# Sukikui/PTI-LDM-VAE

Hardware: AMD Instinct MI355X
Metric: vae_train_images_per_sec_256x256 (higher is better)
Workload: dtype fp16 forward operands + activations / bf16 backward operands + gradients, fp32 accumulate; 1 GPU; config/vae_dente_no_adv.json 256x256x1 batch 32/GPU: fwd + L1 + 1e-3*KL + bwd + all-reduce + Adam (perceptual term omitted: --perceptual times it; adversarial branch inactive before epoch 6, --adv times it); global_batch=32, parallelism=dp1

## Files before the change

pti_ldm_vae_amd/csrc/wgrad_mfma.hip:

```cpp
#include "pti_common.h"

namespace {

constexpr int TH = 8, TW = 16;
constexpr int PTI_WGRAD_SLAB_V4 = 1 << 30;
#ifndef PTI_WGRAD_BATCH_MAX
#define PTI_WGRAD_BATCH_MAX 16
#endif

struct WgArgs {
  const bf16* x;
  const bf16* dy;
  const stat_t* in_stats;
  const float* gamma;
  const float* beta;
  float* slab;
  int N, H, W, Cin, Ho, Wo, Cout;
  int mode, prologue, groups;
  float eps, inv_cnt;
  int tiles_x, tiles_y, ntiles, S;
  int ci_tiles;
  long long slab_stride;
  int x_f16;
  int diag;
};

template <int KS, int S_, int CO_T, int CI_T>
struct WCfg {
  static constexpr int HH = (TH - 1) * S_ + KS, HW = (TW - 1) * S_ + KS;
  static constexpr int NP = HH * HW;
  static constexpr int KK = KS * KS;
  static constexpr int PA = CI_T * 2 + (CI_T == 64 ? 64 : 0);
  static constexpr int PD = CO_T * 2 + (CO_T == 64 ? 64 : 0);
  static constexpr int NCA = CI_T / 8, NCD = CO_T / 8;
  static constexpr int WCO = CO_T / 32, WCI = CI_T / 32, WPX = 4 / (WCO * WCI);
  static constexpr int A_BYTES = NP * PA, D_BYTES = TH * TW * PD;
  static constexpr int HIT = (NP * NCA + 255) / 256, DIT = (TH * TW * NCD + 255) / 256;
  static constexpr int RED_BYTES = (WPX > 1) ? 32 * 32 * 4 * (WPX - 1) * WCO * WCI : 0;
  static constexpr int LDS_BYTES = (A_BYTES + D_BYTES) > RED_BYTES ? (A_BYTES + D_BYTES) : RED_BYTES;
};

template <int KS, int S_, int CO_T, int CI_T, bool PLAIN>
__global__ __launch_bounds__(256, 2) void wgrad_mfma_kernel(WgArgs a) {
  using C = WCfg<KS, S_, CO_T, CI_T>;
  const int prologue = PLAIN ? PTI_PRO_NONE : a.prologue;
  typedef short v4s __attribute__((ext_vector_type(4)));
  __shared__ __attribute__((aligned(16))) unsigned char smem[C::LDS_BYTES];
  unsigned char* lA = smem;
  unsigned char* lD = smem + C::A_BYTES;

  const int tid = threadIdx.x, lane = tid & 63, wave = tid >> 6;
  const int split = blockIdx.y;
// ... 370 lines not shown
#pragma unroll
          for (int h = 0; h < COB; ++h)
            acc[h][kh] = __builtin_amdgcn_mfma_f32_32x32x16_bf16(dfr[h][o], afr, acc[h][kh], 0, 0, 0);
        }
      }
    }
    __syncthreads();
  }

  float* slab = a.slab + (size_t)split * a.slab_stride;
  const int ci = cit * 32 + (lane & 31);
  const int hsel = lane >> 5;
#pragma unroll
  for (int h = 0; h < COB; ++h)
#pragma unroll
    for (int kh = 0; kh < 3; ++kh)
#pragma unroll
      for (int r = 0; r < 16; ++r) {
        const int co = co0 + h * 32 + (r & 3) + 8 * (r >> 2) + 4 * hsel;
        slab[((size_t)(kh * 3 + kw) * a.Cout + co) * a.Cin + ci] = acc[h][kh][r];
      }
  if (cit == 0) {
    float* red = reinterpret_cast<float*>(smem);
#pragma unroll
    for (int j = 0; j < 8; ++j) red[j * C::NT + tid] = bsum[j];
    __syncthreads();
    if (tid < 32 * COB) {
      const int c8 = tid / 8, j = tid % 8;
      float sm = 0.f;
      for (int k = c8; k < C::NT; k += C::DPC) sm += red[j * C::NT + k];
      slab[(size_t)9 * a.Cout * a.Cin + co0 + tid] = sm;
    }
  }
}

__device__ __attribute__((aligned(16))) unsigned int pti_wgrad_zero_page[4] = {0u, 0u, 0u, 0u};

__device__ __forceinline__ void glds16(const void* gsrc, unsigned lds_dst) {
  unsigned keep;
  asm volatile("s_mov_b32 %0, m0\n\ts_mov_b32 m0, %2\n\ts_nop 0\n\tglobal_load_lds_dwordx4 %1, off\n\ts_mov_b32 m0, %0"
               : "=&s"(keep) : "v"(gsrc), "s"(lds_dst) : "memory");
}
template <int N> __device__ __forceinline__ void wait_vmcnt() { asm volatile("s_waitcnt vmcnt(%0)" :: "n"(N) : "memory"); }

constexpr int W4_STG = 20 * 1024, W4_DP = 3, W4_NSTAGE = 2 * (W4_DP + 1), W4_IMG = 9 * 32 * 32 * 4;
constexpr int W4_STG2 = 28 * 1024, W4_DP2 = 4, W4_NST2 = W4_DP2 + 1;
constexpr int W4_LDS = (W4_NSTAGE * W4_STG > 4 * W4_IMG + 1024) ? W4_NSTAGE * W4_STG : 4 * W4_IMG + 1024;

struct W4Job {
  const bf16* x; const bf16* dy; float* slab;
  long long slab_stride;
  int N, H, W, Cin, Cout, tiles_x, tiles_y, ntiles, S;
  int cob2;
};
constexpr int W4_MAXGRP = 64;
struct W4Batch {
  W4Job job[PTI_WGRAD_BATCH_MAX];
  float* dw[PTI_WGRAD_BATCH_MAX];
  float* dbias[PTI_WGRAD_BATCH_MAX];
  int accumulate[PTI_WGRAD_BATCH_MAX];
  int first_rblk[PTI_WGRAD_BATCH_MAX + 1];
  unsigned short grp[8][W4_MAXGRP];
  unsigned short grp_start[8][W4_MAXGRP + 1];
  int ngrp[8];
  int njobs, diag, nwg;
};

static_assert(sizeof(W4Batch) <= 4096 && PTI_WGRAD_BATCH_MAX <= 16, "kernarg limit / 4-bit job index of the group word");

template <bool COB2>
__global__ __launch_bounds__(512, 1) void wgrad_mfma4_kernel(W4Batch b) {
  constexpr int HWp = TW + 2, NPX = 10 * HWp, PP = 64, XB = 12 * 1024, STG = W4_STG, DP = W4_DP, NPS = DP + 1;
  static_assert(W4_LDS <= 160 * 1024 && 5 * (DP - 1) <= 63, "ring must fit the LDS and the vmcnt counter");
  static_assert(W4_NST2 * W4_STG2 <= W4_LDS && 5 * (W4_DP2 - 1) <= 63, "two-block ring must fit as well");
  const int xcd = blockIdx.x & 7, pos = blockIdx.x >> 3;
  const int ng = b.ngrp[xcd];
  if (ng == 0 || pos >= b.grp_start[xcd][ng]) return;
  int gi = 0;
  while (gi + 1 < ng && pos >= b.grp_start[xcd][gi + 1]) ++gi;
  const unsigned gword = b.grp[xcd][gi];
  const int jb = gword & 15, split = gword >> 4, cc = pos - b.grp_start[xcd][gi];
  const W4Job& a = b.job[jb];
  const int ci_tiles = a.Cin / 32;
  typedef short v4s __attribute__((ext_vector_type(4)));
  typedef short v8s __attribute__((ext_vector_type(8)));
  __shared__ __attribute__((aligned(16))) unsigned char smem[W4_LDS];
  const unsigned lds0 = (unsigned)(size_t)(__attribute__((address_space(3))) unsigned char*)smem;
  const int tid = threadIdx.x, lane = tid & 63;
  const int w8 = __builtin_amdgcn_readfirstlane(tid >> 6);
  const int grp = w8 >> 2, w = w8 & 3;
  const int cot = cc / ci_tiles, cit = cc % ci_tiles;
  constexpr bool cob2 = COB2;
  const int co0 = cob2 ? (2 * cot + grp) * 32 : cot * 32, ci0 = cit * 32;
  const bool do_bias = (cit == 0);

  int xhy[3], xhx[3], xrel[3];
#pragma unroll
  for (int k = 0; k < 3; ++k) {
    const int i = (w + 4 * k) * 64 + lane, p = i >> 2;
    xhy[k] = p < NPX ? p / HWp : 1 << 20;
    xhx[k] = p - (p / HWp) * HWp;
    xrel[k] = ((xhy[k] - 1) * a.W + xhx[k] - 1) * a.Cin * 2 + (ci0 + (i & 3) * 8) * 2;
  }
  int dty[2], dtx[2], drel[2];
#pragma unroll
  for (int k = 0; k < 2; ++k) {
// ... 417 lines not shown
    for (int bl = 0; bl < 2; ++bl) {
      const float t = bsum[bl] + __shfl_xor(bsum[bl], 32, 64);
      if (lane < 32) bred[(w * 2 + bl) * 32 + lane] = t;
    }
  }
  if (w >= 2) { dump(red + (2 * (w - 2)) * 9216, 0); dump(red + (2 * (w - 2) + 1) * 9216, 1); }
  __syncthreads();
  if (w < 2) { gather(red + (2 * w) * 9216, 0); gather(red + (2 * w + 1) * 9216, 1); }
  __syncthreads();
  if (w == 1) { dump(red, 0); dump(red + 9216, 1); }
  __syncthreads();
  if (w == 0) { gather(red, 0); gather(red + 9216, 1); }
  __syncthreads();
  if (w == 0) { dump(red, 0); dump(red + 9216, 1); }
  __syncthreads();
  float* slab2 = a.slab + (size_t)split * a.slab_stride + (size_t)(2 * cot * ci_tiles + cit) * 9216;
  for (int i4 = tid; i4 < 2 * 2304; i4 += 256) {
    const int g2 = i4 >= 2304, j4 = i4 - g2 * 2304;
    *(f32x4*)(slab2 + (size_t)g2 * ci_tiles * 9216 + j4 * 4) = *(const f32x4*)(red + g2 * 9216 + j4 * 4);
  }
  if (do_bias && tid < 64) {
    const int g2 = tid >> 5;
    float sm = 0.f;
#pragma unroll
    for (int k = 0; k < 4; ++k) sm += bred[(k * 2 + g2) * 32 + (tid & 31)];
    a.slab[(size_t)split * a.slab_stride + (size_t)9 * a.Cout * a.Cin + cot * 64 + tid] = sm;
  }
#undef AC
}

template <int NCB_, int NCH_, int NRG_>
struct W6Cfg {
  static constexpr int NCB = NCB_, NCH = NCH_, NRG = NRG_, TH_ = 4 * NRG_, HW_ = TW + 2, NPX = (TH_ + 2) * HW_;
  static constexpr int XI = (NPX + 15) / 16;
  static constexpr int XSUB = XI * 1024, XB = NCH * XSUB, DSUB = TH_ * 1024, STG = XB + NCB * DSUB;
  static constexpr int NX = NCH * XI, KX = (NX + 7) / 8, ND = NCB * TH_, KD = ND / 8, NSLOT = KX + KD;
  static constexpr bool SINK = NX % 8 != 0;
  static constexpr int STGS = STG + (SINK ? 1024 : 0);
  static constexpr int FOLD = NRG == 2 ? NCB * NCH * 5 * 1024 * 4 + 1024 : 0;
#ifdef W6_NST3
  static constexpr int NST = 3, DP = 2;
#else
  static constexpr int NST = (124 * 1024) / STGS >= 4 ? 4 : 3, DP = NST - 1;
#endif
  static constexpr int LDS = NST * STGS > FOLD ? NST * STGS : FOLD;
  static_assert(NCB * NCH * NRG == 8 && ND % 8 == 0 && LDS <= 160 * 1024 && NSLOT * (DP - 1) <= 63, "v6 shape");
};
using W6A = W6Cfg<4, 2, 1>;
using W6B = W6Cfg<2, 2, 2>;

#ifndef W6_VGPR_ATTR
#define W6_VGPR_ATTR
#endif
template <class C>
__global__ W6_VGPR_ATTR __launch_bounds__(512, 1) void wgrad_mfma6_kernel(W4Batch b) {
  constexpr int PP = 64, HWp = C::HW_;
  const int xcd = blockIdx.x & 7, pos = blockIdx.x >> 3;
  const int ng = b.ngrp[xcd];
  if (ng == 0 || pos >= b.grp_start[xcd][ng]) return;
  int gi = 0;
  while (gi + 1 < ng && pos >= b.grp_start[xcd][gi + 1]) ++gi;
  const unsigned gword = b.grp[xcd][gi];
  const int jb = gword & 15, split = gword >> 4, cc = pos - b.grp_start[xcd][gi];
  const W4Job& a = b.job[jb];
  const int ci_pairs = a.Cin / (32 * C::NCH);
  typedef short v4s __attribute__((ext_vector_type(4)));
  typedef short v8s __attribute__((ext_vector_type(8)));
  __shared__ __attribute__((aligned(16))) unsigned char smem[C::LDS];
  const unsigned lds0 = (unsigned)(size_t)(__attribute__((address_space(3))) unsigned char*)smem;
  const int tid = threadIdx.x, lane = tid & 63;
  const int w8 = __builtin_amdgcn_readfirstlane(tid >> 6);
  const int cb = w8 % C::NCB, ch = (w8 / C::NCB) % C::NCH, rg = w8 / (C::NCB * C::NCH);
  const int cotb = cc / ci_pairs, citb = cc % ci_pairs;
  const int co0 = cotb * 32 * C::NCB, ci0 = citb * 32 * C::NCH;
  const bool do_bias = (citb == 0) && (ch == 0);

  int H = a.H, W = a.W;
  asm volatile("" : "+s"(H), "+s"(W));
  int ldsoff[C::NSLOT];
  int yy[C::NSLOT], xx[C::NSLOT], rel[C::NSLOT];
  bool pv[C::NSLOT];
  {
    const int pix = lane >> 2, piece = lane & 3;
#pragma unroll
    for (int k = 0; k < C::KX; ++k) {
      const int xi = w8 + 8 * k;
      const bool sink = xi >= C::NX;
      const int h = xi / C::XI, i = xi - C::XI * h, p = 16 * i + pix;
      ldsoff[k] = sink ? C::STG : h * C::XSUB + i * 1024;
      pv[k] = !sink && p < C::NPX;
      yy[k] = p / HWp - 1;
      xx[k] = p - (p / HWp) * HWp - 1;
      rel[k] = (yy[k] * W + xx[k]) * a.Cin * 2 + (ci0 + h * 32 + piece * 8) * 2;
    }
#pragma unroll
    for (int k = C::KX; k < C::NSLOT; ++k) {
      const int di = w8 + 8 * (k - C::KX), c = di / C::TH_, i = di % C::TH_;
      ldsoff[k] = C::XB + c * C::DSUB + i * 1024;
      pv[k] = true;
      yy[k] = i;
      xx[k] = pix;
      rel[k] = (i * W + pix) * a.Cout * 2 + (co0 + c * 32 + piece * 8) * 2;
    }
#pragma unroll
    for (int k = 0; k < C::NSLOT; ++k) ldsoff[k] = __builtin_amdgcn_readfirstlane(ldsoff[k]);
  }
  const unsigned char* xb = reinterpret_cast<const unsigned char*>(a.x);
  const unsigned char* db = reinterpret_cast<const unsigned char*>(a.dy);
  const unsigned char* zero = reinterpret_cast<const unsigned char*>(pti_wgrad_zero_page);
  struct TilePos { const unsigned char* xt; const unsigned char* dt; int oy0, ox0; };
  auto locate = [&](int tile) -> TilePos {
    TilePos tp;
    const bool live = tile < a.ntiles;
    int t = live ? tile : 0;
    const int tx_ = t % a.tiles_x; t /= a.tiles_x;
    const int ty_ = t % a.tiles_y;
    const int n = t / a.tiles_y;
    tp.oy0 = live ? ty_ * C::TH_ : 1 << 24; tp.ox0 = tx_ * TW;
    const size_t pix0 = (size_t)(n * H + ty_ * C::TH_) * W + tp.ox0;
    tp.xt = xb + pix0 * a.Cin * 2;
    tp.dt = db + pix0 * a.Cout * 2;
    return tp;
  };
  auto issue_slot = [&](const TilePos& tp, int stage, int k) {
    if (b.diag & 1) return;
    const unsigned sb = __builtin_amdgcn_readfirstlane(lds0 + stage * C::STGS + ldsoff[k]);
    const bool ok = pv[k] && (unsigned)(tp.oy0 + yy[k]) < (unsigned)H && (unsigned)(tp.ox0 + xx[k]) < (unsigned)W;
    glds16(ok ? (k < C::KX ? tp.xt : tp.dt) + rel[k] : zero, sb);
  };

  f32x16 acc[3][3];
  float bsum = 0.f;
#pragma unroll
  for (int r = 0; r < 16; ++r)
#pragma unroll
    for (int kh = 0; kh < 3; ++kh)
#pragma unroll
      for (int kw = 0; kw < 3; ++kw) acc[kh][kw][r] = 0.f;
  const int g = lane >> 4, q = (lane & 15) >> 2, pp = lane & 3;
  const int fbase = (8 * (g >> 1) + q) * PP + (16 * (g & 1) + 4 * pp) * 2;
  auto tr_frag = [&](const unsigned char* p) -> bf16x8 {
    const v4s d0 = __builtin_amdgcn_ds_read_tr16_b64_v4i16((v4s __attribute__((address_space(3)))*)(p));
    const v4s d1 = __builtin_amdgcn_ds_read_tr16_b64_v4i16((v4s __attribute__((address_space(3)))*)(p + 4 * PP));
    const v8s t = {d0[0], d0[1], d0[2], d0[3], d1[0], d1[1], d1[2], d1[3]};
    return __builtin_bit_cast(bf16x8, t);
  };

  const int ntl = a.ntiles > split ? (a.ntiles - split + a.S - 1) / a.S : 0;
  auto tile_of = [&](int k) { return k < ntl ? split + k * a.S : a.ntiles; };
#pragma unroll
  for (int s = 0; s < C::DP; ++s) {
    const TilePos tp = locate(tile_of(s));
#pragma unroll
    for (int k = 0; k < C::NSLOT; ++k) issue_slot(tp, s, k);
  }
  bf16x8 dfr[4], xcur, xq1;
  auto xfrag_at = [&](const unsigned char* lX, int f) { return tr_frag(lX + fbase + ((4 * rg + f / 3) * HWp + f % 3) * PP); };
  auto dfrag_at = [&](const unsigned char* lS, int r) { return tr_frag(lS + C::XB + cb * C::DSUB + fbase + (4 * rg + r) * TW * PP); };
  wait_vmcnt<C::NSLOT * (C::DP - 1)>();
  __builtin_amdgcn_s_barrier();
#pragma unroll
  for (int r = 0; r < 4; ++r) dfr[r] = dfrag_at(smem, r);
  xcur = xfrag_at(smem + ch * C::XSUB, 0);
  xq1 = xfrag_at(smem + ch * C::XSUB, 1);

  int ps = 0;
  for (int it = 0; it < ntl; ++it) {
    int fs = ps + C::DP;
    fs = fs >= C::NST ? fs - C::NST : fs;
    const int ns = ps + 1 == C::NST ? 0 : ps + 1;
    const TilePos ft = locate(tile_of(it + C::DP));
    wait_vmcnt<C::NSLOT * (C::DP - 2)>();
    __builtin_amdgcn_s_barrier();
    const unsigned char* lX = smem + ps * C::STGS + ch * C::XSUB;
    const unsigned char* lN = smem + ns * C::STGS;
    if (b.diag & 2) {
#pragma unroll
      for (int k = 0; k < C::NSLOT; ++k) issue_slot(ft, fs, k);
      ps = ns;
      continue;
    }
    if (do_bias) {
#pragma unroll
      for (int r = 0; r < 4; ++r) {
        const u32x4 dwv = __builtin_bit_cast(u32x4, dfr[r]);
        float s8 = 0.f;
#pragma unroll
        for (int i = 0; i < 4; ++i) s8 += __uint_as_float(dwv[i] << 16) + __uint_as_float(dwv[i] & 0xffff0000u);
        bsum += s8;
      }
    }
    bf16x8 dnx[4];
#pragma unroll
    for (int f = 0; f < 18; ++f) {
      const int rr = f / 3, kw = f % 3;
      bf16x8 xq2 = f + 2 < 18 ? xfrag_at(lX, f + 2) : xfrag_at(lN + ch * C::XSUB, f + 2 - 18);
      if (kw == 0 && rr >= 2) dnx[rr - 2] = dfrag_at(lN, rr - 2);
#pragma unroll
      for (int kh = 0; kh < 3; ++kh) {
        const int r = rr - kh;
        if (r >= 0 && r < 4) acc[kh][kw] = __builtin_amdgcn_mfma_f32_32x32x16_bf16(dfr[r], xcur, acc[kh][kw], 0, 0, 0);
      }
      if (C::NSLOT == 4) {
        if (f == 2) issue_slot(ft, fs, 0);
        if (f == 6) issue_slot(ft, fs, 1);
        if (f == 10) issue_slot(ft, fs, 2);
        if (f == 14) issue_slot(ft, fs, 3);
      } else {
        if (f == 2) issue_slot(ft, fs, 0);
        if (f == 5) issue_slot(ft, fs, 1);
        if (f == 8) issue_slot(ft, fs, 2);
        if (f == 11) issue_slot(ft, fs, 3);
        if (f == 14) issue_slot(ft, fs, C::NSLOT - 1);
      }
      if (kw == 0 && rr >= 2) __builtin_amdgcn_sched_group_barrier(0x100, 4, 0);
      else __builtin_amdgcn_sched_group_barrier(0x100, 2, 0);
      {
        const int nm = (rr == 0 || rr == 5) ? 1 : ((rr == 1 || rr == 4) ? 2 : 3);
        if (nm == 3) __builtin_amdgcn_sched_group_barrier(0x008, 3, 0);
        else if (nm == 2) __builtin_amdgcn_sched_group_barrier(0x008, 2, 0);
        else __builtin_amdgcn_sched_group_barrier(0x008, 1, 0);
      }
      __builtin_amdgcn_sched_barrier(0);
      xcur = xq1;
      xq1 = xq2;
    }
#pragma unroll
    for (int r = 0; r < 4; ++r) dfr[r] = dnx[r];
    ps = ns;
  }
  wait_vmcnt<0>();

  const int ci = lane & 31, hsel = lane >> 5;
  if (do_bias) bsum += __shfl_xor(bsum, 32, 64);
  if constexpr (C::NRG == 2) {
    __syncthreads();
    float* red = reinterpret_cast<float*>(smem) + (cb + C::NCB * ch) * 5120;
    float* bred = reinterpret_cast<float*>(smem) + C::NCB * C::NCH * 5120;
#pragma unroll
    for (int round = 0; round < 2; ++round) {
      if (round) __syncthreads();
      if (rg == 1) {
#pragma unroll
        for (int t = 0; t < 9; ++t)
          if ((t < 5) == (round == 0))
#pragma unroll
            for (int q4 = 0; q4 < 4; ++q4)
              *(f32x4*)(red + (t - 5 * round) * 1024 + ci * 32 + (((2 * q4 + hsel) ^ (ci & 7)) << 2)) =
                  f32x4{acc[t / 3][t % 3][4 * q4], acc[t / 3][t % 3][4 * q4 + 1], acc[t / 3][t % 3][4 * q4 + 2], acc[t / 3][t % 3][4 * q4 + 3]};
        if (round == 0 && do_bias && lane < 32) bred[cb * 32 + lane] = bsum;
      }
      __syncthreads();
      if (rg == 0) {
#pragma unroll
        for (int t = 0; t < 9; ++t)
          if ((t < 5) == (round == 0))
#pragma unroll
            for (int q4 = 0; q4 < 4; ++q4) {
              const f32x4 v = *(const f32x4*)(red + (t - 5 * round) * 1024 + ci * 32 + (((2 * q4 + hsel) ^ (ci & 7)) << 2));
#pragma unroll
              for (int j = 0; j < 4; ++j) acc[t / 3][t % 3][4 * q4 + j] += v[j];
            }
        if (round == 0 && do_bias && lane < 32) bsum += bred[cb * 32 + lane];
      }
    }
    if (rg == 1) return;
  }
  const int cc32 = (C::NCB * cotb + cb) * (a.Cin / 32) + C::NCH * citb + ch;
  float* blk = a.slab + (size_t)split * a.slab_stride + (size_t)cc32 * 9216;
#pragma unroll
  for (int kh = 0; kh < 3; ++kh)
#pragma unroll
    for (int kw = 0; kw < 3; ++kw)
#pragma unroll
      for (int q4 = 0; q4 < 4; ++q4)
        *(f32x4*)(blk + (kh * 3 + kw) * 1024 + ci * 32 + (((2 * q4 + hsel) ^ (ci & 7)) << 2)) =
            f32x4{acc[kh][kw][4 * q4], acc[kh][kw][4 * q4 + 1], acc[kh][kw][4 * q4 + 2], acc[kh][kw][4 * q4 + 3]};
  if (do_bias && lane < 32) a.slab[(size_t)split * a.slab_stride + (size_t)9 * a.Cout * a.Cin + co0 + cb * 32 + lane] = bsum;
}

__global__ __launch_bounds__(256) void wgrad_reduce4_kernel(W4Batch b) {
  __shared__ f32x4 red[16][16];
  int jb = 0;
  while (jb + 1 < b.njobs && (int)blockIdx.x >= b.first_rblk[jb + 1]) ++jb;
  const W4Job& a = b.job[jb];
  const float* __restrict__ slab = a.slab;
  float* __restrict__ dw = b.dw[jb];
  float* __restrict__ dbias = b.dbias[jb];
  const int S = a.S, Cout = a.Cout, Cin = a.Cin, accumulate = b.accumulate[jb];
  const long long stride = a.slab_stride;
  const long long total = (long long)9 * Cout * Cin;
  const int col = threadIdx.x & 15, sg = threadIdx.x >> 4;
  const long long e = ((long long)(blockIdx.x - b.first_rblk[jb]) * 16 + col) * 4;
  f32x4 s0 = {0.f, 0.f, 0.f, 0.f}, s1 = s0;
  if (e < total + Cout) {
    int k = sg;
    for (; k + 16 < S; k += 32) {
      s0 += *(const f32x4*)(slab + (size_t)k * stride + e);
      s1 += *(const f32x4*)(slab + (size_t)(k + 16) * stride + e);
    }
    if (k < S) s0 += *(const f32x4*)(slab + (size_t)k * stride + e);
  }
  red[sg][col] = s0 + s1;
  __syncthreads();
  if (sg == 0 && e < total + Cout) {
    f32x4 sum = red[0][col];
#pragma unroll
    for (int g = 1; g < 16; ++g) sum += red[g][col];
    if (e < total) {
      const int cc = (int)(e / 9216), i = (int)(e % 9216);
      const int ci_tiles = Cin / 32;
      const int co0 = (cc / ci_tiles) * 32, ci0 = (cc % ci_tiles) * 32;
      const int tap = i >> 10, ci = (i >> 5) & 31, cog = ((i >> 2) & 7) ^ (ci & 7);
#pragma unroll
      for (int j = 0; j < 4; ++j) {
        const size_t o = ((size_t)(co0 + cog * 4 + j) * Cin + ci0 + ci) * 9 + tap;
        dw[o] = accumulate ? dw[o] + sum[j] : sum[j];
      }
    } else if (dbias) {
      const int co = (int)(e - total);
#pragma unroll
      for (int j = 0; j < 4; ++j) dbias[co + j] = accumulate ? dbias[co + j] + sum[j] : sum[j];
    }
  }
}

__global__ __launch_bounds__(256) void wgrad_reduce_kernel(const float* __restrict__ slab, long long stride, int S,
                                                           float* __restrict__ dw, float* __restrict__ dbias, int Cout,
                                                           int Cin, int KK, int accumulate) {
  __shared__ f32x4 red[16][16];
// ... 6 lines not shown
    for (; k + 16 < S; k += 32) {
      s0 += *(const f32x4*)(slab + (size_t)k * stride + e);
      s1 += *(const f32x4*)(slab + (size_t)(k + 16) * stride + e);
    }
    if (k < S) s0 += *(const f32x4*)(slab + (size_t)k * stride + e);
  }
  red[sg][col] = s0 + s1;
  __syncthreads();
  if (sg == 0 && e < total + Cout) {
    f32x4 sum = red[0][col];
#pragma unroll
    for (int g = 1; g < 16; ++g) sum += red[g][col];
    if (e < total) {
      const int ci = e % Cin;
      const int co = (e / Cin) % Cout;
      const int t = e / ((long long)Cin * Cout);
#pragma unroll
      for (int j = 0; j < 4; ++j) {
        const size_t o = ((size_t)co * Cin + ci + j) * KK + t;
        dw[o] = accumulate ? dw[o] + sum[j] : sum[j];
      }
    } else if (dbias) {
      const int co = (int)(e - total);
#pragma unroll
      for (int j = 0; j < 4; ++j) dbias[co + j] = accumulate ? dbias[co + j] + sum[j] : sum[j];
    }
  }
}

template <int KS, int S_, int CO_T, int CI_T>
void launch_w(const WgArgs& a, int grid_y, hipStream_t st) {
  if (a.prologue == PTI_PRO_NONE)
    PTI_LAUNCH((wgrad_mfma_kernel<KS, S_, CO_T, CI_T, true>), dim3(grid_y, a.S), dim3(256), 0, st, a);
  else
    PTI_LAUNCH((wgrad_mfma_kernel<KS, S_, CO_T, CI_T, false>), dim3(grid_y, a.S), dim3(256), 0, st, a);
}
template <int KS, int S_>
void launch_wt(const WgArgs& a, int co_t, int ci_t, int grid_y, hipStream_t st) {
  if (co_t == 64 && ci_t == 64) launch_w<KS, S_, 64, 64>(a, grid_y, st);
  else if (co_t == 64) launch_w<KS, S_, 64, 32>(a, grid_y, st);
  else if (ci_t == 64) launch_w<KS, S_, 32, 64>(a, grid_y, st);
  else launch_w<KS, S_, 32, 32>(a, grid_y, st);
}

}

static int w6_mode(int n, int h, int w, int cin, int cout) {
  const char* e = getenv("PTI_WGRAD_V6");
  const int v = e ? atoi(e) : 3;
  if (v >= 1 && cout % 128 == 0 && cin % 64 == 0) return 2;
  if (v >= 2 && cout % 64 == 0 && cin % 64 == 0 && (v == 2 || (long long)h * w <= 128 * 128)) return 3;
  return 0;
}
static void w4_fill_job(W4Job& a, const void* x, const void* dy, int n, int h, int w, int cin, int cout, int v6 = 0) {
  a.x = (const bf16*)x; a.dy = (const bf16*)dy; a.slab = nullptr;
  a.N = n; a.H = h; a.W = w; a.Cin = cin; a.Cout = cout;
  a.tiles_x = cdiv(w, TW); a.tiles_y = cdiv(h, v6 == 2 ? W6A::TH_ : TH); a.ntiles = n * a.tiles_x * a.tiles_y;
  a.slab_stride = (long long)9 * cout * cin + cout;
  a.S = 1;
  static const int cob2_env = getenv("PTI_WGRAD_V4_COB2") ? atoi(getenv("PTI_WGRAD_V4_COB2")) : 1;
  a.cob2 = v6 ? v6 : ((cob2_env && cout % 64 == 0) ? 1 : 0);
}
static bool w4_eligible(int n, int h, int w, int cin, int cout) {
  return n > 0 && h > 0 && w > 0 && cin > 0 && cout > 0 && cin % 32 == 0 && cout % 32 == 0 &&
         (long long)n * h * w * cin * 2 < (1ll << 31) && (long long)n * h * w * cout * 2 < (1ll << 31);
}
static int wgrad_diag_env() {
  const char* v = getenv("PTI_WGRAD_V4_DIAG");
  const char* ok = getenv("PTI_ALLOW_WRONG_RESULTS");
  if (!v || atoi(v) == 0) return 0;
  if (!ok || atoi(ok) != 1) {
    fprintf(stderr, "[pti] PTI_WGRAD_V4_DIAG ignored: it needs PTI_ALLOW_WRONG_RESULTS=1 (results are garbage)\n");
    return 0;
  }
  fprintf(stderr, "[pti] WRONG-RESULT DIAGNOSTIC ACTIVE: PTI_WGRAD_V4_DIAG=%s\n", v);
  return atoi(v);
}
static long long w4_plan(W4Batch& b, float* workspace, long long workspace_floats) {
  static const int wgs_env = getenv("PTI_WGRAD_V4_WGS") ? atoi(getenv("PTI_WGRAD_V4_WGS")) : 2048;
  static const int diag_env = wgrad_diag_env();
  b.diag = diag_env;
  auto tiles32 = [](const W4Job& a) {
    return a.cob2 == 2 ? (a.Cin / 64) * (a.Cout / 128) : a.cob2 == 3 ? (a.Cin / 64) * (a.Cout / 64)
                                                                     : (a.Cin / 32) * (a.Cout / (a.cob2 ? 64 : 32));
  };
  const bool m6 = b.njobs > 0 && b.job[0].cob2 >= 2;
  const char* w6e = getenv("PTI_WGRAD_V6_WGS");
  const int wgs6 = w6e && atoi(w6e) > 0 ? atoi(w6e) : 512;
  double work = 0;
  for (int j = 0; j < b.njobs; ++j) work += (double)tiles32(b.job[j]) * (b.job[j].cob2 == 1 ? 2 : 1) * b.job[j].ntiles;
  double per_wg = work / wgs_env > 2.0 ? work / wgs_env : 2.0;
  if (m6) per_wg = work / wgs6 > 4.0 ? work / wgs6 : 4.0;
  for (int attempt = 0;; ++attempt) {
    long long used = 0;
    int rb = 0, groups = 0;
    bool fits = true;
    for (int j = 0; j < b.njobs; ++j) {
      W4Job& a = b.job[j];
      int S = (int)((double)a.ntiles * (a.cob2 == 1 ? 2 : 1) / per_wg + 0.5);
      if (S > a.ntiles / (a.cob2 ? 1 : 2)) S = a.ntiles / (a.cob2 ? 1 : 2);
      if (S > 255) S = 255;
      if (S < 1) S = 1;
      if (used + (long long)S * a.slab_stride > workspace_floats) fits = false;
      a.S = S;
      a.slab = workspace + used;
      used += (long long)S * a.slab_stride;
      groups += S;
      b.first_rblk[j] = rb;
      rb += (int)((a.slab_stride / 4 + 15) / 16);
    }
    b.first_rblk[b.njobs] = rb;
    if (fits && groups <= 8 * W4_MAXGRP) {
      int len[8] = {0, 0, 0, 0, 0, 0, 0, 0};
      for (int x = 0; x < 8; ++x) { b.ngrp[x] = 0; b.grp_start[x][0] = 0; }
      int order[PTI_WGRAD_BATCH_MAX];
      for (int j = 0; j < b.njobs; ++j) order[j] = j;
      for (int i = 0; i < b.njobs; ++i)
        for (int j = i + 1; j < b.njobs; ++j)
          if (tiles32(b.job[order[j]]) > tiles32(b.job[order[i]])) { const int t = order[i]; order[i] = order[j]; order[j] = t; }
      bool ok = true;
      for (int i = 0; i < b.njobs && ok; ++i) {
        const int j = order[i];
        for (int sp = 0; sp < b.job[j].S; ++sp) {
          int best = 0;
          for (int x = 1; x < 8; ++x)
            if (len[x] < len[best]) best = x;
          if (b.ngrp[best] >= W4_MAXGRP || len[best] + tiles32(b.job[j]) > 65535) { ok = false; break; }
          b.grp[best][b.ngrp[best]] = (unsigned short)((unsigned)j | ((unsigned)sp << 4));
          len[best] += tiles32(b.job[j]);
          b.grp_start[best][++b.ngrp[best]] = (unsigned short)len[best];
        }
      }
      if (ok) {
        int mx = 0;
        for (int x = 0; x < 8; ++x) mx = len[x] > mx ? len[x] : mx;
        b.nwg = 8 * mx;
        return used;
      }
    }
    if (attempt > 40) return -1;
    per_wg *= 1.25;
  }
}

extern "C" int64_t pti_conv_wgrad_workspace_bytes(int cout, int cin, int ksize, int splits) {
  return (int64_t)splits * ((int64_t)ksize * ksize * cout * cin + cout) * 4;
}

static int wgrad_check(const void* x, const void* dy, const int64_t* in_stats, const float* gamma, const float* beta,
                       const void* workspace, const pti_conv_desc* d) {
  if (!x || !dy || !workspace || !d) PTI_FAIL(PTI_EINVAL, "conv_wgrad_mfma: null pointer");
  if (d->cin % 32 || d->cout % 32) PTI_FAIL(PTI_EUNSUPPORTED, "conv_wgrad_mfma: cin=%d cout=%d", d->cin, d->cout);
  if (d->ksize != 1 && d->ksize != 3) PTI_FAIL(PTI_EUNSUPPORTED, "conv_wgrad_mfma: ksize");
  if (d->mode == PTI_CONV_ZINS || (d->ksize == 1 && d->mode != PTI_CONV_S1)) PTI_FAIL(PTI_EUNSUPPORTED, "conv_wgrad_mfma: mode %d", d->mode);
  if (d->prologue != PTI_PRO_NONE && (!in_stats || !gamma || !beta || d->groups <= 0 || d->cin % d->groups))
    PTI_FAIL(PTI_EINVAL, "conv_wgrad_mfma: prologue args");
  return PTI_OK;
}

extern "C" int pti_conv_wgrad_mfma_partials(const void* x, const void* dy, const int64_t* in_stats, const float* gamma,
                                            const float* beta, void* workspace, int64_t workspace_bytes,
                                            const pti_conv_desc* d, int* splits_out, pti_stream_t s) {
  if (!splits_out) PTI_FAIL(PTI_EINVAL, "conv_wgrad_mfma_partials: null splits_out");
  if (int rc = wgrad_check(x, dy, in_stats, gamma, beta, workspace, d)) return rc;
  WgArgs a;
  a.x = (const bf16*)x; a.dy = (const bf16*)dy; a.in_stats = (const stat_t*)in_stats; a.gamma = gamma; a.beta = beta;
  a.slab = (float*)workspace;
  a.N = d->n; a.H = d->h; a.W = d->w; a.Cin = d->cin; a.Ho = d->ho; a.Wo = d->wo; a.Cout = d->cout;
  a.mode = d->mode; a.prologue = d->prologue; a.groups = d->groups; a.eps = d->eps; a.x_f16 = d->in_f16;
  static const int diag_env = wgrad_diag_env();
  a.diag = diag_env;
  a.inv_cnt = d->prologue != PTI_PRO_NONE ? 1.0f / ((float)(d->cin / d->groups) * (float)d->h * (float)d->w) : 0.f;
  a.tiles_x = cdiv(d->wo, TW); a.tiles_y = cdiv(d->ho, TH); a.ntiles = d->n * a.tiles_x * a.tiles_y;
  int co_t = d->cout % 64 == 0 ? 64 : 32, ci_t = d->cin % 64 == 0 ? 64 : 32;
  if ((long long)a.ntiles * (d->cout / co_t) * (d->cin / ci_t) < 16 * 512) co_t = ci_t = 32;
  const bool v3 = d->ksize == 3 && d->mode != PTI_CONV_S2PAD;
  static const int cob_env = getenv("PTI_WGRAD_COB") ? atoi(getenv("PTI_WGRAD_COB")) : 0;
  const bool cob_ok = d->cout % 64 == 0 && d->mode == PTI_CONV_S1;
  const int cob = (cob_ok && cob_env != 1 && (cob_env == 2 || d->prologue != PTI_PRO_NONE)) ? 2 : 1;
  if (v3) { ci_t = 32; co_t = 32 * cob; }
  a.ci_tiles = d->cin / ci_t;
  const int tiles_cc = (d->cout / co_t) * a.ci_tiles;
  const int kk = d->ksize * d->ksize;
  a.slab_stride = (long long)kk * d->cout * d->cin + d->cout;
  const long long smax = workspace_bytes / (a.slab_stride * 4);
  const bool plain = d->prologue == PTI_PRO_NONE && cob == 1;
  static const int v1_wgs = getenv("PTI_WGRAD_V1_WGS") ? atoi(getenv("PTI_WGRAD_V1_WGS")) : 512;
  int S = (v3 ? (cob == 2 ? 512 : (plain ? (tiles_cc == 1 ? 1024 : 1280) : 768)) : v1_wgs) / tiles_cc;
  if (S > a.ntiles / 4) S = a.ntiles / 4;
  const int scap = v3 ? (plain ? 1024 : 512) : 256;
  if (S > scap) S = scap;
  if (S < 1) S = 1;
  if (S > smax) S = (int)smax;
  if (S < 1) PTI_FAIL(PTI_EINVAL, "conv_wgrad_mfma: workspace too small (%lld bytes per split needed)", a.slab_stride * 4);
  static const int v4_env = getenv("PTI_WGRAD_V4") ? atoi(getenv("PTI_WGRAD_V4")) : 1;
  const bool v4 = v3 && v4_env && d->prologue == PTI_PRO_NONE && !d->in_f16 && d->mode == PTI_CONV_S1 &&
                  w4_eligible(d->n, d->h, d->w, d->cin, d->cout);
  if (v4) {
    W4Batch b;
    b.njobs = 1;
    w4_fill_job(b.job[0], x, dy, d->n, d->h, d->w, d->cin, d->cout, w6_mode(d->n, d->h, d->w, d->cin, d->cout));
    b.dw[0] = b.dbias[0] = nullptr;
    b.accumulate[0] = 0;
    if (w4_plan(b, (float*)workspace, workspace_bytes / 4) < 0)
      PTI_FAIL(PTI_EINVAL, "conv_wgrad_mfma: workspace too small (%lld bytes per split needed)", a.slab_stride * 4);
    const char* v5e = getenv("PTI_WGRAD_V5");
    const bool v5 = v5e && atoi(v5e) != 0 && !b.diag;
    if (b.job[0].cob2 == 2) PTI_LAUNCH(wgrad_mfma6_kernel<W6A>, dim3(b.nwg), dim3(512), 0, (hipStream_t)s, b);
    else if (b.job[0].cob2 == 3) PTI_LAUNCH(wgrad_mfma6_kernel<W6B>, dim3(b.nwg), dim3(512), 0, (hipStream_t)s, b);
    else if (b.job[0].cob2 && v5) PTI_LAUNCH(wgrad_mfma5_kernel, dim3(b.nwg), dim3(256), 0, (hipStream_t)s, b);
    else if (b.job[0].cob2) PTI_LAUNCH(wgrad_mfma4_kernel<true>, dim3(b.nwg), dim3(512), 0, (hipStream_t)s, b);
    else PTI_LAUNCH(wgrad_mfma4_kernel<false>, dim3(b.nwg), dim3(512), 0, (hipStream_t)s, b);
    PTI_CHECK_LAUNCH("conv_wgrad_mfma");
    *splits_out = b.job[0].S | PTI_WGRAD_SLAB_V4;
    return PTI_OK;
  }
  if (v3 && S >= 8) S &= ~7;
  a.S = S;
  hipStream_t st = (hipStream_t)s;
  if (v3 && cob == 2) PTI_LAUNCH((wgrad_mfma3_kernel<2, false>), dim3(tiles_cc * S), dim3(192), 0, st, a);
  else if (v3 && plain) PTI_LAUNCH((wgrad_mfma3_kernel<1, true>), dim3(tiles_cc * S), dim3(192), 0, st, a);
  else if (v3) PTI_LAUNCH((wgrad_mfma3_kernel<1, false>), dim3(tiles_cc * S), dim3(192), 0, st, a);
  else if (d->ksize == 1) launch_wt<1, 1>(a, co_t, ci_t, tiles_cc, st);
  else launch_wt<3, 2>(a, co_t, ci_t, tiles_cc, st);
  PTI_CHECK_LAUNCH("conv_wgrad_mfma");
  *splits_out = S;
  return PTI_OK;
}

extern "C" int pti_conv_wgrad_reduce(const void* workspace, int splits, float* dw, float* dbias, int accumulate,
                                     const pti_conv_desc* d, pti_stream_t s) {
  if (!workspace || !dw || !d || splits < 1) PTI_FAIL(PTI_EINVAL, "conv_wgrad_reduce: bad arguments");
  const int kk = d->ksize * d->ksize;
  const long long total = (long long)kk * d->cout * d->cin + d->cout;
  if (splits & PTI_WGRAD_SLAB_V4) {
    if (kk != 9 || !w4_eligible(d->n, d->h, d->w, d->cin, d->cout)) PTI_FAIL(PTI_EINVAL, "conv_wgrad_reduce: block-ordered slabs are 3x3 only");
    W4Batch b;
    b.njobs = 1;
    w4_fill_job(b.job[0], nullptr, nullptr, d->n, d->h, d->w, d->cin, d->cout);
    b.job[0].S = splits & ~PTI_WGRAD_SLAB_V4;
    b.job[0].slab = (float*)workspace;
    b.dw[0] = dw; b.dbias[0] = dbias; b.accumulate[0] = accumulate;
    b.diag = 0; b.nwg = 0;
    for (int x = 0; x < 8; ++x) b.ngrp[x] = 0;
    b.first_rblk[0] = 0;
    b.first_rblk[1] = (int)((total / 4 + 15) / 16);
    PTI_LAUNCH(wgrad_reduce4_kernel, dim3(b.first_rblk[1]), dim3(256), 0, (hipStream_t)s, b);
    PTI_CHECK_LAUNCH("conv_wgrad_reduce");
    return PTI_OK;
  }
  PTI_LAUNCH(wgrad_reduce_kernel, dim3((unsigned)((total / 4 + 15) / 16)), dim3(256), 0, (hipStream_t)s,
                     (const float*)workspace, total, splits, dw, dbias, d->cout, d->cin, kk, accumulate);
  PTI_CHECK_LAUNCH("conv_wgrad_reduce");
  return PTI_OK;
}

extern "C" int pti_conv_wgrad_mfma(const void* x, const void* dy, const int64_t* in_stats, const float* gamma,
                                   const float* beta, float* dw, float* dbias, void* workspace,
                                   int64_t workspace_bytes, int accumulate, const pti_conv_desc* d, pti_stream_t s) {
  if (!dw) PTI_FAIL(PTI_EINVAL, "conv_wgrad_mfma: null pointer");
  int splits = 0;
  if (int rc = pti_conv_wgrad_mfma_partials(x, dy, in_stats, gamma, beta, workspace, workspace_bytes, d, &splits, s)) return rc;
  return pti_conv_wgrad_reduce(workspace, splits, dw, dbias, accumulate, d, s);
}

extern "C" int pti_conv_wgrad_mfma_batched(const pti_wgrad_job* jobs, int njobs, void* workspace, int64_t workspace_bytes,
                                           pti_stream_t s) {
  if (!jobs || !workspace || njobs < 1 || njobs > PTI_WGRAD_BATCH_MAX)
    PTI_FAIL(PTI_EINVAL, "conv_wgrad_mfma_batched: 1..%d jobs", PTI_WGRAD_BATCH_MAX);
  W4Batch bm[4];
  bm[0].njobs = bm[1].njobs = bm[2].njobs = bm[3].njobs = 0;
  for (int j = 0; j < njobs; ++j) {
    const pti_wgrad_job& q = jobs[j];
    if (!q.x || !q.dy || !q.dw) PTI_FAIL(PTI_EINVAL, "conv_wgrad_mfma_batched: job %d has a null pointer", j);
    if (!w4_eligible(q.n, q.h, q.w, q.cin, q.cout))
      PTI_FAIL(PTI_EUNSUPPORTED, "conv_wgrad_mfma_batched: job %d: n=%d h=%d w=%d cin=%d cout=%d (channels must be multiples of 32, tensors < 2 GiB)",
               j, q.n, q.h, q.w, q.cin, q.cout);
    W4Job jb;
    w4_fill_job(jb, q.x, q.dy, q.n, q.h, q.w, q.cin, q.cout, w6_mode(q.n, q.h, q.w, q.cin, q.cout));
    W4Batch& b = bm[jb.cob2];
    const int k = b.njobs++;
    b.job[k] = jb;
    b.dw[k] = q.dw; b.dbias[k] = q.dbias; b.accumulate[k] = q.accumulate;
  }
  float* ws = (float*)workspace;
  long long ws_floats = workspace_bytes / 4;
  const char* v5e = getenv("PTI_WGRAD_V5");
  const int v5_env = v5e ? atoi(v5e) : 0;
  const void* main_kernel = nullptr;
  long long need[4] = {0, 0, 0, 0}, need_all = 0;
  for (int m = 0; m < 4; ++m) {
    for (int j = 0; j < bm[m].njobs; ++j) need[m] += bm[m].job[j].slab_stride;
    need_all += need[m];
  }
  if (need_all > ws_floats) PTI_FAIL(PTI_EINVAL, "conv_wgrad_mfma_batched: workspace too small (%lld bytes needed for one split per job)", need_all * 4);
  const long long ws_total = ws_floats;
  for (int m = 3; m >= 0; --m) {
    W4Batch& b = bm[m];
    if (b.njobs == 0) continue;
    long long later = 0;
    for (int m2 = m - 1; m2 >= 0; --m2) later += need[m2];
    long long avail = (long long)((double)ws_total * ((double)need[m] / (double)need_all));
    if (avail < need[m]) avail = need[m];
    if (later == 0 || avail > ws_floats - later) avail = ws_floats - later;
    const long long used = w4_plan(b, ws, avail);
    if (used < 0) PTI_FAIL(PTI_EINVAL, "conv_wgrad_mfma_batched: workspace too small");
    ws += used;
    ws_floats -= used;
    const void* kfn;
    if (m == 3) { PTI_LAUNCH(wgrad_mfma6_kernel<W6B>, dim3(b.nwg), dim3(512), 0, (hipStream_t)s, b); kfn = reinterpret_cast<const void*>(wgrad_mfma6_kernel<W6B>); }
    else if (m == 2) { PTI_LAUNCH(wgrad_mfma6_kernel<W6A>, dim3(b.nwg), dim3(512), 0, (hipStream_t)s, b); kfn = reinterpret_cast<const void*>(wgrad_mfma6_kernel<W6A>); }
    else if (m == 1 && v5_env && !b.diag) { PTI_LAUNCH(wgrad_mfma5_kernel, dim3(b.nwg), dim3(256), 0, (hipStream_t)s, b); kfn = reinterpret_cast<const void*>(wgrad_mfma5_kernel); }
    else if (m == 1) { PTI_LAUNCH(wgrad_mfma4_kernel<true>, dim3(b.nwg), dim3(512), 0, (hipStream_t)s, b); kfn = reinterpret_cast<const void*>(wgrad_mfma4_kernel<true>); }
    else { PTI_LAUNCH(wgrad_mfma4_kernel<false>, dim3(b.nwg), dim3(512), 0, (hipStream_t)s, b); kfn = reinterpret_cast<const void*>(wgrad_mfma4_kernel<false>); }
    PTI_CHECK_LAUNCH("conv_wgrad_mfma_batched");
    if (!main_kernel) main_kernel = kfn;
    PTI_LAUNCH(wgrad_reduce4_kernel, dim3(b.first_rblk[b.njobs]), dim3(256), 0, (hipStream_t)s, b);
    PTI_CHECK_LAUNCH("conv_wgrad_mfma_batched reduce");
  }
  pti_last_kernel = main_kernel;
  return PTI_OK;
}
```

Baseline: 2693 images/s.

## Add polyphase nearest-upsample wgrad path to MFMA v6 kernel

Adds an UP2 variant of the v6 MFMA weight-gradient kernel for convolutions that follow a 2x nearest upsample. Each split now handles one of the four output phases, and the 3x3 taps collapse into a 2x2 accumulator set. The kernel reads the low-resolution input directly instead of the upsampled tensor, which cuts MFMA work and input traffic. The accumulators are scattered back into 3x3 slab taps per phase so the existing reduce kernel can sum them, and the planner's split count and workgroup count are adjusted for the fourfold phase parallelism. The costs are extra phase splits in the slab workspace and a more complex scheduling pattern.

```diff
diff --git a/pti_ldm_vae_amd/csrc/wgrad_mfma.hip b/pti_ldm_vae_amd/csrc/wgrad_mfma.hip
--- a/pti_ldm_vae_amd/csrc/wgrad_mfma.hip
+++ b/pti_ldm_vae_amd/csrc/wgrad_mfma.hip
@@ -1,3 +1,4 @@
+#include <type_traits>
 #include "pti_common.h"
 
 namespace {
@@ -474,6 +475,7 @@
   long long slab_stride;
   int N, H, W, Cin, Cout, tiles_x, tiles_y, ntiles, S;
   int cob2;
+  int up2;
 };
 constexpr int W4_MAXGRP = 64;
 struct W4Batch {
@@ -997,9 +999,10 @@
 #ifndef W6_VGPR_ATTR
 #define W6_VGPR_ATTR
 #endif
-template <class C>
+template <class C, bool UP2>
 __global__ W6_VGPR_ATTR __launch_bounds__(512, 1) void wgrad_mfma6_kernel(W4Batch b) {
   constexpr int PP = 64, HWp = C::HW_;
+  constexpr int NT = UP2 ? 2 : 3, NF = (NT + 3) * NT, DS = UP2 ? 2 : 1;
   const int xcd = blockIdx.x & 7, pos = blockIdx.x >> 3;
   const int ng = b.ngrp[xcd];
   if (ng == 0 || pos >= b.grp_start[xcd][ng]) return;
@@ -1009,6 +1012,8 @@
   const int jb = gword & 15, split = gword >> 4, cc = pos - b.grp_start[xcd][gi];
   const W4Job& a = b.job[jb];
   const int ci_pairs = a.Cin / (32 * C::NCH);
+  const int py = UP2 ? (split >> 1) & 1 : 0, px = UP2 ? split & 1 : 0;
+  const int tsplit = UP2 ? split >> 2 : split, tS = UP2 ? a.S >> 2 : a.S;
   typedef short v4s __attribute__((ext_vector_type(4)));
   typedef short v8s __attribute__((ext_vector_type(8)));
   __shared__ __attribute__((aligned(16))) unsigned char smem[C::LDS];
@@ -1045,7 +1050,7 @@
       pv[k] = true;
       yy[k] = i;
       xx[k] = pix;
-      rel[k] = (i * W + pix) * a.Cout * 2 + (co0 + c * 32 + piece * 8) * 2;
+      rel[k] = (i * W * (DS * DS) + pix * DS) * a.Cout * 2 + (co0 + c * 32 + piece * 8) * 2;
     }
 #pragma unroll
     for (int k = 0; k < C::NSLOT; ++k) ldsoff[k] = __builtin_amdgcn_readfirstlane(ldsoff[k]);
@@ -1064,7 +1069,8 @@
     tp.oy0 = live ? ty_ * C::TH_ : 1 << 24; tp.ox0 = tx_ * TW;
     const size_t pix0 = (size_t)(n * H + ty_ * C::TH_) * W + tp.ox0;
     tp.xt = xb + pix0 * a.Cin * 2;
-    tp.dt = db + pix0 * a.Cout * 2;
+    if constexpr (UP2) tp.dt = db + ((size_t)(2 * (n * H + ty_ * C::TH_) + py) * (2 * W) + 2 * tp.ox0 + px) * a.Cout * 2;
+    else tp.dt = db + pix0 * a.Cout * 2;
     return tp;
   };
   auto issue_slot = [&](const TilePos& tp, int stage, int k) {
@@ -1074,16 +1080,17 @@
     glds16(ok ? (k < C::KX ? tp.xt : tp.dt) + rel[k] : zero, sb);
   };
 
-  f32x16 acc[3][3];
+  f32x16 acc[NT][NT];
   float bsum = 0.f;
 #pragma unroll
   for (int r = 0; r < 16; ++r)
 #pragma unroll
-    for (int kh = 0; kh < 3; ++kh)
-#pragma unroll
-      for (int kw = 0; kw < 3; ++kw) acc[kh][kw][r] = 0.f;
+    for (int kh = 0; kh < NT; ++kh)
+#pragma unroll
+      for (int kw = 0; kw < NT; ++kw) acc[kh][kw][r] = 0.f;
   const int g = lane >> 4, q = (lane & 15) >> 2, pp = lane & 3;
   const int fbase = (8 * (g >> 1) + q) * PP + (16 * (g & 1) + 4 * pp) * 2;
+  const int fbx = fbase + (py * HWp + px) * PP;
   auto tr_frag = [&](const unsigned char* p) -> bf16x8 {
     const v4s d0 = __builtin_amdgcn_ds_read_tr16_b64_v4i16((v4s __attribute__((address_space(3)))*)(p));
     const v4s d1 = __builtin_amdgcn_ds_read_tr16_b64_v4i16((v4s __attribute__((address_space(3)))*)(p + 4 * PP));
@@ -1091,8 +1098,8 @@
     return __builtin_bit_cast(bf16x8, t);
   };
 
-  const int ntl = a.ntiles > split ? (a.ntiles - split + a.S - 1) / a.S : 0;
-  auto tile_of = [&](int k) { return k < ntl ? split + k * a.S : a.ntiles; };
+  const int ntl = a.ntiles > tsplit ? (a.ntiles - tsplit + tS - 1) / tS : 0;
+  auto tile_of = [&](int k) { return k < ntl ? tsplit + k * tS : a.ntiles; };
 #pragma unroll
   for (int s = 0; s < C::DP; ++s) {
     const TilePos tp = locate(tile_of(s));
@@ -1100,7 +1107,7 @@
     for (int k = 0; k < C::NSLOT; ++k) issue_slot(tp, s, k);
   }
   bf16x8 dfr[4], xcur, xq1;
-  auto xfrag_at = [&](const unsigned char* lX, int f) { return tr_frag(lX + fbase + ((4 * rg + f / 3) * HWp + f % 3) * PP); };
+  auto xfrag_at = [&](const unsigned char* lX, int f) { return tr_frag(lX + fbx + ((4 * rg + f / NT) * HWp + f % NT) * PP); };
   auto dfrag_at = [&](const unsigned char* lS, int r) { return tr_frag(lS + C::XB + cb * C::DSUB + fbase + (4 * rg + r) * TW * PP); };
   wait_vmcnt<C::NSLOT * (C::DP - 1)>();
   __builtin_amdgcn_s_barrier();
@@ -1137,16 +1144,20 @@
     }
     bf16x8 dnx[4];
 #pragma unroll
-    for (int f = 0; f < 18; ++f) {
-      const int rr = f / 3, kw = f % 3;
-      bf16x8 xq2 = f + 2 < 18 ? xfrag_at(lX, f + 2) : xfrag_at(lN + ch * C::XSUB, f + 2 - 18);
-      if (kw == 0 && rr >= 2) dnx[rr - 2] = dfrag_at(lN, rr - 2);
-#pragma unroll
-      for (int kh = 0; kh < 3; ++kh) {
+    for (int f = 0; f < NF; ++f) {
+      const int rr = f / NT, kw = f % NT;
+      bf16x8 xq2 = f + 2 < NF ? xfrag_at(lX, f + 2) : xfrag_at(lN + ch * C::XSUB, f + 2 - NF);
+      if (kw == 0 && rr >= NT - 1) dnx[rr - (NT - 1)] = dfrag_at(lN, rr - (NT - 1));
+#pragma unroll
+      for (int kh = 0; kh < NT; ++kh) {
         const int r = rr - kh;
         if (r >= 0 && r < 4) acc[kh][kw] = __builtin_amdgcn_mfma_f32_32x32x16_bf16(dfr[r], xcur, acc[kh][kw], 0, 0, 0);
       }
-      if (C::NSLOT == 4) {
+      if constexpr (UP2) {
+#pragma unroll
+        for (int k = 0; k < C::NSLOT; ++k)
+          if (f == 2 * k + 1) issue_slot(ft, fs, k);
+      } else if (C::NSLOT == 4) {
         if (f == 2) issue_slot(ft, fs, 0);
         if (f == 6) issue_slot(ft, fs, 1);
         if (f == 10) issue_slot(ft, fs, 2);
@@ -1158,10 +1169,10 @@
         if (f == 11) issue_slot(ft, fs, 3);
         if (f == 14) issue_slot(ft, fs, C::NSLOT - 1);
       }
-      if (kw == 0 && rr >= 2) __builtin_amdgcn_sched_group_barrier(0x100, 4, 0);
+      if (kw == 0 && rr >= NT - 1) __builtin_amdgcn_sched_group_barrier(0x100, 4, 0);
       else __builtin_amdgcn_sched_group_barrier(0x100, 2, 0);
       {
-        const int nm = (rr == 0 || rr == 5) ? 1 : ((rr == 1 || rr == 4) ? 2 : 3);
+        const int nm = UP2 ? ((rr == 0 || rr == 4) ? 1 : 2) : (rr == 0 || rr == 5) ? 1 : ((rr == 1 || rr == 4) ? 2 : 3);
         if (nm == 3) __builtin_amdgcn_sched_group_barrier(0x008, 3, 0);
         else if (nm == 2) __builtin_amdgcn_sched_group_barrier(0x008, 2, 0);
         else __builtin_amdgcn_sched_group_barrier(0x008, 1, 0);
@@ -1187,24 +1198,24 @@
       if (round) __syncthreads();
       if (rg == 1) {
 #pragma unroll
-        for (int t = 0; t < 9; ++t)
+        for (int t = 0; t < NT * NT; ++t)
           if ((t < 5) == (round == 0))
 #pragma unroll
             for (int q4 = 0; q4 < 4; ++q4)
               *(f32x4*)(red + (t - 5 * round) * 1024 + ci * 32 + (((2 * q4 + hsel) ^ (ci & 7)) << 2)) =
-                  f32x4{acc[t / 3][t % 3][4 * q4], acc[t / 3][t % 3][4 * q4 + 1], acc[t / 3][t % 3][4 * q4 + 2], acc[t / 3][t % 3][4 * q4 + 3]};
+                  f32x4{acc[t / NT][t % NT][4 * q4], acc[t / NT][t % NT][4 * q4 + 1], acc[t / NT][t % NT][4 * q4 + 2], acc[t / NT][t % NT][4 * q4 + 3]};
         if (round == 0 && do_bias && lane < 32) bred[cb * 32 + lane] = bsum;
       }
       __syncthreads();
       if (rg == 0) {
 #pragma unroll
-        for (int t = 0; t < 9; ++t)
+        for (int t = 0; t < NT * NT; ++t)
           if ((t < 5) == (round == 0))
 #pragma unroll
             for (int q4 = 0; q4 < 4; ++q4) {
               const f32x4 v = *(const f32x4*)(red + (t - 5 * round) * 1024 + ci * 32 + (((2 * q4 + hsel) ^ (ci & 7)) << 2));
 #pragma unroll
-              for (int j = 0; j < 4; ++j) acc[t / 3][t % 3][4 * q4 + j] += v[j];
+              for (int j = 0; j < 4; ++j) acc[t / NT][t % NT][4 * q4 + j] += v[j];
             }
         if (round == 0 && do_bias && lane < 32) bsum += bred[cb * 32 + lane];
       }
@@ -1213,14 +1224,26 @@
   }
   const int cc32 = (C::NCB * cotb + cb) * (a.Cin / 32) + C::NCH * citb + ch;
   float* blk = a.slab + (size_t)split * a.slab_stride + (size_t)cc32 * 9216;
-#pragma unroll
-  for (int kh = 0; kh < 3; ++kh)
-#pragma unroll
-    for (int kw = 0; kw < 3; ++kw)
-#pragma unroll
-      for (int q4 = 0; q4 < 4; ++q4)
-        *(f32x4*)(blk + (kh * 3 + kw) * 1024 + ci * 32 + (((2 * q4 + hsel) ^ (ci & 7)) << 2)) =
-            f32x4{acc[kh][kw][4 * q4], acc[kh][kw][4 * q4 + 1], acc[kh][kw][4 * q4 + 2], acc[kh][kw][4 * q4 + 3]};
+  auto store_taps = [&](auto PY, auto PX) {
+    constexpr int py_ = decltype(PY)::value, px_ = decltype(PX)::value;
+#pragma unroll
+    for (int kh = 0; kh < 3; ++kh)
+#pragma unroll
+      for (int kw = 0; kw < 3; ++kw) {
+        const f32x16& v = UP2 ? acc[(kh + 1 - py_) >> 1][(kw + 1 - px_) >> 1] : acc[kh % NT][kw % NT];
+#pragma unroll
+        for (int q4 = 0; q4 < 4; ++q4)
+          *(f32x4*)(blk + (kh * 3 + kw) * 1024 + ci * 32 + (((2 * q4 + hsel) ^ (ci & 7)) << 2)) =
+              f32x4{v[4 * q4], v[4 * q4 + 1], v[4 * q4 + 2], v[4 * q4 + 3]};
+      }
+  };
+  typedef std::integral_constant<int, 0> I0;
+  typedef std::integral_constant<int, 1> I1;
+  if constexpr (!UP2) store_taps(I0{}, I0{});
+  else if (py == 0 && px == 0) store_taps(I0{}, I0{});
+  else if (py == 0) store_taps(I0{}, I1{});
+  else if (px == 0) store_taps(I1{}, I0{});
+  else store_taps(I1{}, I1{});
   if (do_bias && lane < 32) a.slab[(size_t)split * a.slab_stride + (size_t)9 * a.Cout * a.Cin + co0 + cb * 32 + lane] = bsum;
 }
 
@@ -1333,7 +1356,7 @@
   if (v >= 2 && cout % 64 == 0 && cin % 64 == 0 && (v == 2 || (long long)h * w <= 128 * 128)) return 3;
   return 0;
 }
-static void w4_fill_job(W4Job& a, const void* x, const void* dy, int n, int h, int w, int cin, int cout, int v6 = 0) {
+static void w4_fill_job(W4Job& a, const void* x, const void* dy, int n, int h, int w, int cin, int cout, int v6 = 0, int up2 = 0) {
   a.x = (const bf16*)x; a.dy = (const bf16*)dy; a.slab = nullptr;
   a.N = n; a.H = h; a.W = w; a.Cin = cin; a.Cout = cout;
   a.tiles_x = cdiv(w, TW); a.tiles_y = cdiv(h, v6 == 2 ? W6A::TH_ : TH); a.ntiles = n * a.tiles_x * a.tiles_y;
@@ -1341,6 +1364,7 @@
   a.S = 1;
   static const int cob2_env = getenv("PTI_WGRAD_V4_COB2") ? atoi(getenv("PTI_WGRAD_V4_COB2")) : 1;
   a.cob2 = v6 ? v6 : ((cob2_env && cout % 64 == 0) ? 1 : 0);
+  a.up2 = up2;
 }
 static bool w4_eligible(int n, int h, int w, int cin, int cout) {
   return n > 0 && h > 0 && w > 0 && cin > 0 && cout > 0 && cin % 32 == 0 && cout % 32 == 0 &&
@@ -1367,9 +1391,10 @@
   };
   const bool m6 = b.njobs > 0 && b.job[0].cob2 >= 2;
   const char* w6e = getenv("PTI_WGRAD_V6_WGS");
-  const int wgs6 = w6e && atoi(w6e) > 0 ? atoi(w6e) : 512;
+  const int wgs6 = w6e && atoi(w6e) > 0 ? atoi(w6e) : (b.njobs > 0 && b.job[0].up2 ? 256 : 512);
   double work = 0;
-  for (int j = 0; j < b.njobs; ++j) work += (double)tiles32(b.job[j]) * (b.job[j].cob2 == 1 ? 2 : 1) * b.job[j].ntiles;
+  for (int j = 0; j < b.njobs; ++j)
+    work += (double)tiles32(b.job[j]) * (b.job[j].cob2 == 1 ? 2 : 1) * (b.job[j].up2 ? 4 : 1) * b.job[j].ntiles;
   double per_wg = work / wgs_env > 2.0 ? work / wgs_env : 2.0;
   if (m6) per_wg = work / wgs6 > 4.0 ? work / wgs6 : 4.0;
   for (int attempt = 0;; ++attempt) {
@@ -1378,10 +1403,12 @@
     bool fits = true;
     for (int j = 0; j < b.njobs; ++j) {
       W4Job& a = b.job[j];
-      int S = (int)((double)a.ntiles * (a.cob2 == 1 ? 2 : 1) / per_wg + 0.5);
-      if (S > a.ntiles / (a.cob2 ? 1 : 2)) S = a.ntiles / (a.cob2 ? 1 : 2);
+      const int par = a.up2 ? 4 : 1;
+      int S = (int)((double)a.ntiles * par * (a.cob2 == 1 ? 2 : 1) / per_wg + 0.5);
+      if (S > a.ntiles * par / (a.cob2 ? 1 : 2)) S = a.ntiles * par / (a.cob2 ? 1 : 2);
       if (S > 255) S = 255;
-      if (S < 1) S = 1;
+      if (a.up2) S &= ~3;
+      if (S < par) S = par;
       if (used + (long long)S * a.slab_stride > workspace_floats) fits = false;
       a.S = S;
       a.slab = workspace + used;
@@ -1477,18 +1504,25 @@
   static const int v4_env = getenv("PTI_WGRAD_V4") ? atoi(getenv("PTI_WGRAD_V4")) : 1;
   const bool v4 = v3 && v4_env && d->prologue == PTI_PRO_NONE && !d->in_f16 && d->mode == PTI_CONV_S1 &&
                   w4_eligible(d->n, d->h, d->w, d->cin, d->cout);
-  if (v4) {
+  const int up2_mode = (v3 && v4_env && d->mode == PTI_CONV_UP2 && d->prologue == PTI_PRO_NONE && !d->in_f16 &&
+                        w4_eligible(d->n, d->h, d->w, d->cin, d->cout) && w4_eligible(d->n, d->ho, d->wo, d->cin, d->cout) &&
+                        d->ho == 2 * d->h && d->wo == 2 * d->w)
+                           ? w6_mode(d->n, d->h, d->w, d->cin, d->cout) : 0;
+  if (v4 || up2_mode) {
     W4Batch b;
     b.njobs = 1;
-    w4_fill_job(b.job[0], x, dy, d->n, d->h, d->w, d->cin, d->cout, w6_mode(d->n, d->h, d->w, d->cin, d->cout));
+    w4_fill_job(b.job[0], x, dy, d->n, d->h, d->w, d->cin, d->cout,
+                up2_mode ? up2_mode : w6_mode(d->n, d->h, d->w, d->cin, d->cout), up2_mode != 0);
     b.dw[0] = b.dbias[0] = nullptr;
     b.accumulate[0] = 0;
     if (w4_plan(b, (float*)workspace, workspace_bytes / 4) < 0)
       PTI_FAIL(PTI_EINVAL, "conv_wgrad_mfma: workspace too small (%lld bytes per split needed)", a.slab_stride * 4);
     const char* v5e = getenv("PTI_WGRAD_V5");
     const bool v5 = v5e && atoi(v5e) != 0 && !b.diag;
-    if (b.job[0].cob2 == 2) PTI_LAUNCH(wgrad_mfma6_kernel<W6A>, dim3(b.nwg), dim3(512), 0, (hipStream_t)s, b);
-    else if (b.job[0].cob2 == 3) PTI_LAUNCH(wgrad_mfma6_kernel<W6B>, dim3(b.nwg), dim3(512), 0, (hipStream_t)s, b);
+    if (up2_mode == 2) PTI_LAUNCH((wgrad_mfma6_kernel<W6A, true>), dim3(b.nwg), dim3(512), 0, (hipStream_t)s, b);
+    else if (up2_mode == 3) PTI_LAUNCH((wgrad_mfma6_kernel<W6B, true>), dim3(b.nwg), dim3(512), 0, (hipStream_t)s, b);
+    else if (b.job[0].cob2 == 2) PTI_LAUNCH((wgrad_mfma6_kernel<W6A, false>), dim3(b.nwg), dim3(512), 0, (hipStream_t)s, b);
+    else if (b.job[0].cob2 == 3) PTI_LAUNCH((wgrad_mfma6_kernel<W6B, false>), dim3(b.nwg), dim3(512), 0, (hipStream_t)s, b);
     else if (b.job[0].cob2 && v5) PTI_LAUNCH(wgrad_mfma5_kernel, dim3(b.nwg), dim3(256), 0, (hipStream_t)s, b);
     else if (b.job[0].cob2) PTI_LAUNCH(wgrad_mfma4_kernel<true>, dim3(b.nwg), dim3(512), 0, (hipStream_t)s, b);
     else PTI_LAUNCH(wgrad_mfma4_kernel<false>, dim3(b.nwg), dim3(512), 0, (hipStream_t)s, b);
@@ -1589,8 +1623,8 @@
     ws += used;
     ws_floats -= used;
     const void* kfn;
-    if (m == 3) { PTI_LAUNCH(wgrad_mfma6_kernel<W6B>, dim3(b.nwg), dim3(512), 0, (hipStream_t)s, b); kfn = reinterpret_cast<const void*>(wgrad_mfma6_kernel<W6B>); }
-    else if (m == 2) { PTI_LAUNCH(wgrad_mfma6_kernel<W6A>, dim3(b.nwg), dim3(512), 0, (hipStream_t)s, b); kfn = reinterpret_cast<const void*>(wgrad_mfma6_kernel<W6A>); }
+    if (m == 3) { PTI_LAUNCH((wgrad_mfma6_kernel<W6B, false>), dim3(b.nwg), dim3(512), 0, (hipStream_t)s, b); kfn = reinterpret_cast<const void*>(wgrad_mfma6_kernel<W6B, false>); }
+    else if (m == 2) { PTI_LAUNCH((wgrad_mfma6_kernel<W6A, false>), dim3(b.nwg), dim3(512), 0, (hipStream_t)s, b); kfn = reinterpret_cast<const void*>(wgrad_mfma6_kernel<W6A, false>); }
     else if (m == 1 && v5_env && !b.diag) { PTI_LAUNCH(wgrad_mfma5_kernel, dim3(b.nwg), dim3(256), 0, (hipStream_t)s, b); kfn = reinterpret_cast<const void*>(wgrad_mfma5_kernel); }
     else if (m == 1) { PTI_LAUNCH(wgrad_mfma4_kernel<true>, dim3(b.nwg), dim3(512), 0, (hipStream_t)s, b); kfn = reinterpret_cast<const void*>(wgrad_mfma4_kernel<true>); }
     else { PTI_LAUNCH(wgrad_mfma4_kernel<false>, dim3(b.nwg), dim3(512), 0, (hipStream_t)s, b); kfn = reinterpret_cast<const void*>(wgrad_mfma4_kernel<false>); }
```

New measurement: 2695 images/s (median of 3 runs). Within noise of the previous version (+0.1%).
